# opendilab/DI-engine

Measured on NVIDIA H100. Metric: learner transitions/sec (GAE+ppo_error fwd+bwd, T=128 x B=4096 per GPU), higher is better.
Workload: dtype f32

## Files before the change

### di-engine_b200/csrc/policy.cu

```cuda
#include <math.h>

#include "../../include/b200rl.h"
#include "policy_stats.cuh"

namespace b200rl {

constexpr int GS_NT = 1024;
constexpr int GS_MAX_T = 24576;

template <int VN>
__global__ void __launch_bounds__(GS_NT) gae_seq_kernel(const float* __restrict__ value, float* __restrict__ next_value,
                                                       const float* __restrict__ reward, const float* __restrict__ done,
                                                       const float* __restrict__ traj, float* __restrict__ adv, int T,
                                                       float gamma, float gl, int mask_inplace, RetArgs ra) {
    pdl_prologue();
    extern __shared__ float s_seq[];
    float* s_d = s_seq;
    float* s_f = s_seq + T;
    __shared__ int s_nseg;
    __shared__ int s_cnt[GS_NT / 32];
    const int tid = threadIdx.x;
    const float vs = ra.vscale;
    float mu = 0.f, sigma = 1.f;
    if constexpr (VN == VN_POPART) {
        mu = *ra.mu;
        sigma = *ra.sigma;
    }
    for (int t = tid; t < T; t += GS_NT) {
        const float v = vn_decode<VN>(value[t], vs);
        float nv = vn_decode<VN>(next_value[t], vs);
        float r = reward[t];
        if constexpr (VN == VN_POPART) r = __fdiv_rn(fsub(r, mu), sigma);
        const float d = done ? done[t] : 0.f;
        const float tf = traj ? traj[t] : d;
        if (done) {
            nv = fmul(nv, fsub(1.f, d));
            if (VN == VN_PPO && mask_inplace && d != 0.f) next_value[t] = nv;
        }
        s_d[t] = fsub(fadd(r, fmul(gamma, nv)), v);
        s_f[t] = fmul(gl, fsub(1.f, tf));
    }
    __syncthreads();
    const int strip = (T + GS_NT - 1) / GS_NT;
    const int t0 = tid * strip, t1 = min(T, t0 + strip);
    int mine = 0;
    for (int t = t0; t < t1; ++t) mine += (s_f[t] == 0.f || t == T - 1) ? 1 : 0;
    int incl = mine;
    const int lane = tid & 31, wid = tid >> 5;
#pragma unroll
    for (int o = 1; o < 32; o <<= 1) {
        const int n = __shfl_up_sync(0xffffffffu, incl, o);
        if (lane >= o) incl += n;
    }
    if (lane == 31) s_cnt[wid] = incl;
    __syncthreads();
    if (wid == 0) {
        int w = s_cnt[lane];
#pragma unroll
        for (int o = 1; o < 32; o <<= 1) {
            const int n = __shfl_up_sync(0xffffffffu, w, o);
            if (lane >= o) w += n;
        }
        s_cnt[lane] = w;
        if (lane == 31) s_nseg = w;
    }
    __syncthreads();
    const int base = incl - mine + (wid ? s_cnt[wid - 1] : 0);
    __shared__ int s_end[GS_NT];
    const int nseg = s_nseg;
    const bool fits = nseg <= GS_NT;
    if (fits) {
        int k = base;
        for (int t = t0; t < t1; ++t)
            if (s_f[t] == 0.f || t == T - 1) s_end[k++] = t;
    }
    __syncthreads();
    if (fits) {
        if (tid < nseg) {
            const int hi = s_end[tid];
            const int lo = tid ? s_end[tid - 1] + 1 : 0;
            float carry = 0.f;
            int t = hi;
            for (; t - 15 >= lo; t -= 16) {
                float d[16], f[16];
#pragma unroll
                for (int k = 0; k < 16; ++k) {
                    d[k] = s_d[t - k];
                    f[k] = s_f[t - k];
                }
#pragma unroll
                for (int k = 0; k < 16; ++k) {
                    carry = fadd(d[k], fmul(f[k], carry));
                    d[k] = carry;
                }
#pragma unroll
                for (int k = 0; k < 16; ++k) s_d[t - k] = d[k];
            }
            for (; t >= lo; --t) {
                carry = fadd(s_d[t], fmul(s_f[t], carry));
                s_d[t] = carry;
            }
        }
    } else if (tid == 0) {
        float carry = 0.f;
        for (int t = T - 1; t >= 0; --t) {
            carry = fadd(s_d[t], fmul(s_f[t], carry));
            s_d[t] = carry;
        }
    }
    __syncthreads();
    if constexpr (VN != VN_PPO) {
        __shared__ int s_cut;
        if (tid == 0) s_cut = -1;
        __syncthreads();
        int cut = -1;
        for (int t = tid; t < T - 1; t += GS_NT)
            if (s_f[t] == 0.f && !isfinite(s_d[t + 1])) cut = t;
        if (cut >= 0) atomicMax(&s_cut, cut);
        __syncthreads();
        const int c = s_cut;
        for (int t = tid; t <= c; t += GS_NT) s_d[t] = __int_as_float(0x7fc00000);
        __syncthreads();
    }
    double acc[4] = {0.0, 0.0, 0.0, 0.0}, pv[2];
    ret_pivots<VN>(vs, vn_decode<VN>(ld_after_wait(value), vs), s_d[0], pv);
    for (int t = tid; t < T; t += GS_NT) {
        const float a = s_d[t];
        adv[t] = a;
        moments_add(acc[2], acc[3], a, pv[1]);
        if (ra.ret_unnorm || ra.value_out || ra.ret_out || ra.stats) {
            float ru, vo, ro;
            moments_add(acc[0], acc[1], ret_encode<VN>(vs, vn_decode<VN>(value[t], vs), a, ru, vo, ro), pv[0]);
            if (ra.ret_unnorm) ra.ret_unnorm[t] = ru;
            if (ra.value_out) ra.value_out[t] = vo;
            if (ra.ret_out) ra.ret_out[t] = ro;
        }
    }
    if (ra.stats || ra.adv_stats) {
        double tot[4];
        if (stats_grid_join<4, GS_NT>(acc, tot, nullptr, nullptr)) write_ret_stats<VN>(ra, tot, pv, (double)T);
    }
}

template <int VN, bool VEC>
__global__ void __launch_bounds__(256) returns_kernel(const float* __restrict__ value, const float* __restrict__ adv,
                                                      long long n, RetArgs ra, double* __restrict__ ws_part,
                                                      unsigned int* __restrict__ ws_join) {
    pdl_prologue();
    const float vs = ra.vscale;
    double acc[4] = {0.0, 0.0, 0.0, 0.0}, pv[2];
    const long long stride = (long long)gridDim.x * 256;
    long long i = (long long)blockIdx.x * 256 + threadIdx.x;
    if (VEC) {
        const long long n4 = n >> 2;
        const float4* v4 = reinterpret_cast<const float4*>(value);
        const float4* a4 = reinterpret_cast<const float4*>(adv);
        float4 v = make_float4(0.f, 0.f, 0.f, 0.f), a = v;
        if (i < n4) {
            v = v4[i];
            a = a4[i];
        }
        ret_pivots<VN>(vs, ret_value<VN>(ld_after_wait(value), vs), ld_after_wait(adv), pv);
        for (; i < n4; i += stride) {
            float4 ru, vo, ro;
            ret_one<VN>(vs, v.x, a.x, ru.x, vo.x, ro.x, acc, pv);
            ret_one<VN>(vs, v.y, a.y, ru.y, vo.y, ro.y, acc, pv);
            ret_one<VN>(vs, v.z, a.z, ru.z, vo.z, ro.z, acc, pv);
            ret_one<VN>(vs, v.w, a.w, ru.w, vo.w, ro.w, acc, pv);
            if (ra.ret_unnorm) reinterpret_cast<float4*>(ra.ret_unnorm)[i] = ru;
            if (ra.value_out) reinterpret_cast<float4*>(ra.value_out)[i] = vo;
            if (ra.ret_out) reinterpret_cast<float4*>(ra.ret_out)[i] = ro;
            if (i + stride < n4) {
                v = v4[i + stride];
                a = a4[i + stride];
            }
        }
    } else {
        float v = 0.f, a = 0.f;
        if (i < n) {
            v = value[i];
            a = adv[i];
        }
        ret_pivots<VN>(vs, ret_value<VN>(ld_after_wait(value), vs), ld_after_wait(adv), pv);
        for (; i < n; i += stride) {
            float ru, vo, ro;
            ret_one<VN>(vs, v, a, ru, vo, ro, acc, pv);
            if (ra.ret_unnorm) ra.ret_unnorm[i] = ru;
            if (ra.value_out) ra.value_out[i] = vo;
            if (ra.ret_out) ra.ret_out[i] = ro;
            if (i + stride < n) {
                v = value[i + stride];
                a = adv[i + stride];
            }
        }
    }
    if (!ra.stats && !ra.adv_stats) return;
    double tot[4];
    if (stats_grid_join<4, 256>(acc, tot, ws_part, ws_join)) write_ret_stats<VN>(ra, tot, pv, (double)n);
}

__global__ void __launch_bounds__(256) adv_stats_kernel(const float* __restrict__ x, long long n, float* __restrict__ out,
                                                        double* __restrict__ ws_part, unsigned int* __restrict__ ws_join) {
    pdl_prologue();
    const double p = stats_pivot(ld_after_wait(x));
    double acc[2] = {0.0, 0.0};
    for (long long i = (long long)blockIdx.x * 256 + threadIdx.x; i < n; i += (long long)gridDim.x * 256)
        moments_add(acc[0], acc[1], x[i], p);
    double tot[2];
    if (stats_grid_join<2, 256>(acc, tot, ws_part, ws_join)) write_adv_stats(out, tot[0], tot[1], p, (double)n);
}

__global__ void __launch_bounds__(256) normalize_kernel(const float* __restrict__ x, const float* __restrict__ stats,
                                                        long long n, float* __restrict__ out) {
    pdl_prologue();
    const float m = ld_after_wait(stats), d = ld_after_wait(stats + 1);
    for (long long i = (long long)blockIdx.x * 256 + threadIdx.x; i < n; i += (long long)gridDim.x * 256)
        out[i] = __fdiv_rn(fsub(x[i], m), d);
}

__global__ void __launch_bounds__(256) impala_mask_kernel(const float* __restrict__ values, const float* __restrict__ rewards,
                                                          const float* __restrict__ done, long long T, long long B,
                                                          float* __restrict__ values_out, float* __restrict__ rewards_out,
                                                          float* __restrict__ weights_out) {
    pdl_prologue();
    const long long n = (T + 1) * B;
    for (long long i = (long long)blockIdx.x * 256 + threadIdx.x; i < n; i += (long long)gridDim.x * 256) {
        const long long t = i / B;
        const float m = t >= 1 ? fsub(1.f, done[i - B]) : 1.f;
        values_out[i] = t >= 1 ? fmul(values[i], m) : values[i];
        if (t < T) {
            if (weights_out) weights_out[i] = m;
            if (rewards_out) rewards_out[i] = fmul(rewards[i], m);
        }
    }
}

enum ValueMap : int { VM_SYMLOG = 0, VM_INV_SYMLOG = 1, VM_H_INV = 2, VM_POPART_REWARD = 3 };

template <int M>
__device__ __forceinline__ float value_map(float x, float mu, float sigma) {
    if constexpr (M == VM_SYMLOG) return vn_symlog(x);
    else if constexpr (M == VM_INV_SYMLOG) return vn_inv_symlog(x);
    else if constexpr (M == VM_H_INV) return vn_h_inv(x);
    else return __fdiv_rn(fsub(x, mu), sigma);
}

template <int M>
__global__ void __launch_bounds__(256) value_map_kernel(const float* __restrict__ x0, float* __restrict__ y0,
                                                        const float* __restrict__ x1, float* __restrict__ y1, long long n,
                                                        const float* __restrict__ mu, const float* __restrict__ sigma) {
    pdl_prologue();
    float m = 0.f, sg = 1.f;
    if constexpr (M == VM_POPART_REWARD) {
        m = *mu;
        sg = *sigma;
    }
    for (long long i = (long long)blockIdx.x * 256 + threadIdx.x; i < n; i += (long long)gridDim.x * 256) {
        y0[i] = value_map<M>(x0[i], m, sg);
        if (x1) y1[i] = value_map<M>(x1[i], m, sg);
    }
}

template <int M>
__global__ void __launch_bounds__(256) value_map_bwd_kernel(const float* __restrict__ x, const float* __restrict__ g,
                                                            float* __restrict__ dx, long long n) {
    pdl_prologue();
    for (long long i = (long long)blockIdx.x * 256 + threadIdx.x; i < n; i += (long long)gridDim.x * 256) {
        const float xi = x[i], s = vn_sign(xi), gs = fmul(g[i], s);
        const float d = M == VM_SYMLOG ? __fdiv_rn(gs, fadd(fabsf(xi), 1.f)) : fmul(gs, expf(fabsf(xi)));
        dx[i] = fadd(0.f, fmul(d, s));
    }
}

}

using namespace b200rl;

namespace b200rl {
int gae_scan(const float* value, float* next_value, const float* reward, const float* done, const float* traj_flag, float* adv,
             long long T, long long C, long long A, double gamma_d, double lambda_d, int mask_next_value_inplace,
             float vscale, void* stream);
}

static double* ws_stats_part(float* ws) { return reinterpret_cast<double*>(ws + WS_CTRL_WORDS); }
static unsigned int* ws_joins(float* ws) { return reinterpret_cast<unsigned int*>(ws + WS_FX_OFF_WORDS + 48); }
static_assert(WS_CTRL_WORDS % 2 == 0 && WS_CTRL_WORDS + NUM_SMS * 8 * 4 * 2 <= WS_PARTIAL_LIMIT_WORDS,
              "the statistics rows fit the workspace's partial region");

extern "C" int b200rl_adv_stats(const float* x, long long n, float* stats2, float* workspace, size_t workspace_bytes,
                                void* stream) {
    if (!x || !stats2 || !workspace || n < 1 || workspace_bytes < WS_MIN_BYTES) return B200RL_ERR_ARG;
    long long grid = div_up(n, 256 * 8);
    if (grid > NUM_SMS * 4) grid = NUM_SMS * 4;
    if (grid < 1) grid = 1;
    return launch_k(adv_stats_kernel, (int)grid, 256, 0, (cudaStream_t)stream, x, n, stats2, ws_stats_part(workspace),
                    ws_joins(workspace));
}

extern "C" int b200rl_normalize(const float* x, const float* stats2, long long n, float* out, void* stream) {
    if (!x || !stats2 || !out || n < 0) return B200RL_ERR_ARG;
    if (n == 0) return B200RL_OK;
    long long grid = div_up(n, 256 * 4);
    if (grid > NUM_SMS * 8) grid = NUM_SMS * 8;
    return launch_k(normalize_kernel, (int)grid, 256, 0, (cudaStream_t)stream, x, stats2, n, out);
}

extern "C" int b200rl_gae_returns(const float* value, float* next_value, const float* reward, const float* done,
                                  const float* traj_flag, long long T, long long C, long long A, double gamma,
                                  double lambda_, int mask_next_value_inplace, double value_scale, float* adv,
                                  float* unnormalized_return, float* value_out, float* return_out, float* stats3,
                                  float* adv_stats2, float* workspace, size_t workspace_bytes, void* stream) {
    if (T < 1 || C < 1 || A < 1 || !value || !next_value || !reward || !adv || !workspace ||
        workspace_bytes < WS_MIN_BYTES || value_scale < 0.0)
        return B200RL_ERR_ARG;
    RetArgs ra{};
    ra.vscale = (float)value_scale;
    ra.ret_unnorm = unnormalized_return; ra.value_out = value_out; ra.ret_out = return_out; ra.stats = stats3;
    ra.adv_stats = adv_stats2;
    cudaStream_t st = (cudaStream_t)stream;
    if (C == 1 && T <= GS_MAX_T) {
        const size_t smem = (size_t)2 * T * sizeof(float);
        if (int rc = smem_opt_in<gae_seq_kernel<VN_PPO>>(smem)) return rc;
        return launch_k(gae_seq_kernel<VN_PPO>, 1, GS_NT, smem, st, value, next_value, reward, done, traj_flag, adv, (int)T,
                        (float)gamma, (float)(gamma * lambda_), mask_next_value_inplace, ra);
    }
    const bool want_epi = unnormalized_return || value_out || return_out || stats3 || adv_stats2;
    int rc = gae_scan(value, next_value, reward, done, traj_flag, adv, T, C, A, gamma, lambda_, mask_next_value_inplace,
                      (float)value_scale, stream);
    if (rc != 0 || !want_epi) return rc;
    const long long n = T * C;
    const bool vec = (n % 4 == 0) && aligned16(value) && aligned16(adv) && (!unnormalized_return || aligned16(unnormalized_return)) &&
                     (!value_out || aligned16(value_out)) && (!return_out || aligned16(return_out));
    long long grid = div_up(n, 256 * (vec ? 8 : 4));
    if (grid > NUM_SMS * 8) grid = NUM_SMS * 8;
    if (vec)
        return launch_k(returns_kernel<VN_PPO, true>, (int)grid, 256, 0, st, value, (const float*)adv, n, ra,
                        ws_stats_part(workspace), ws_joins(workspace));
    return launch_k(returns_kernel<VN_PPO, false>, (int)grid, 256, 0, st, value, (const float*)adv, n, ra,
                    ws_stats_part(workspace), ws_joins(workspace));
}

static long long map_grid(long long n) {
    long long grid = div_up(n, 256 * 4);
    if (grid > NUM_SMS * 8) grid = NUM_SMS * 8;
    return grid < 1 ? 1 : grid;
}

template <int VN>
static int launch_gae_seq(const float* value, const float* next_value, const float* reward, const float* done,
                          const float* traj_flag, float* adv, long long T, double gamma, double lambda_, const RetArgs& ra,
                          cudaStream_t st) {
    const size_t smem = (size_t)2 * T * sizeof(float);
    if (int rc = smem_opt_in<gae_seq_kernel<VN>>(smem)) return rc;
    return launch_k(gae_seq_kernel<VN>, 1, GS_NT, smem, st, value, const_cast<float*>(next_value), reward, done, traj_flag,
                    adv, (int)T, (float)gamma, (float)(gamma * lambda_), 0, ra);
}

template <int VN>
static int launch_returns(const float* value, const float* adv, long long n, const RetArgs& ra, float* workspace,
                          cudaStream_t st) {
    const bool vec = (n % 4 == 0) && aligned16(value) && aligned16(adv) && (!ra.value_out || aligned16(ra.value_out)) &&
                     (!ra.ret_out || aligned16(ra.ret_out));
    long long grid = div_up(n, 256 * (vec ? 8 : 4));
    if (grid > NUM_SMS * 8) grid = NUM_SMS * 8;
    if (vec)
        return launch_k(returns_kernel<VN, true>, (int)grid, 256, 0, st, value, adv, n, ra, ws_stats_part(workspace),
                        ws_joins(workspace));
    return launch_k(returns_kernel<VN, false>, (int)grid, 256, 0, st, value, adv, n, ra, ws_stats_part(workspace),
                    ws_joins(workspace));
}

template <int VN>
static int launch_gae_returns_tc(const float* value, const float* next_value, const float* reward, const float* done,
                                 const float* traj_flag, float* adv, long long T, long long C, double gamma, double lambda_,
                                 const RetArgs& ra, float* scratch, float* workspace, cudaStream_t st) {
    const long long n = T * C;
    const float* v = value;
    const float* nv = next_value;
    const float* r = reward;
    int rc = 0;
    if constexpr (VN == VN_RESCALE || VN == VN_SYMLOG) {
        constexpr int M = VN == VN_RESCALE ? VM_H_INV : VM_INV_SYMLOG;
        rc = launch_k(value_map_kernel<M>, (int)map_grid(n), 256, 0, st, value, scratch, next_value, scratch + n, n,
                      (const float*)nullptr, (const float*)nullptr);
        v = scratch;
        nv = scratch + n;
    } else if constexpr (VN == VN_POPART) {
        rc = launch_k(value_map_kernel<VM_POPART_REWARD>, (int)map_grid(n), 256, 0, st, reward, scratch,
                      (const float*)nullptr, (float*)nullptr, n, ra.mu, ra.sigma);
        r = scratch;
    }
    if (rc) return rc;
    rc = gae_scan(v, const_cast<float*>(nv), r, done, traj_flag, adv, T, C, 1, gamma, lambda_, 0,
                  VN == VN_BASELINE ? ra.vscale : 0.f, st);
    if (rc || !(ra.value_out || ra.ret_out || ra.stats || ra.adv_stats)) return rc;
    return launch_returns<VN>(v, adv, n, ra, workspace, st);
}

template <int VN>
static int gae_returns_norm(const float* value, const float* next_value, const float* reward, const float* done,
                            const float* traj_flag, float* adv, long long T, long long C, double gamma, double lambda_,
                            const RetArgs& ra, float* scratch, float* workspace, cudaStream_t st) {
    if (C == 1 && T <= GS_MAX_T)
        return launch_gae_seq<VN>(value, next_value, reward, done, traj_flag, adv, T, gamma, lambda_, ra, st);
    return launch_gae_returns_tc<VN>(value, next_value, reward, done, traj_flag, adv, T, C, gamma, lambda_, ra, scratch,
                                     workspace, st);
}

extern "C" int b200rl_gae_returns_norm(const float* value, const float* next_value, const float* reward, const float* done,
                                       const float* traj_flag, long long T, long long C, double gamma, double lambda_,
                                       int value_norm, double std, const float* popart_mu, const float* popart_sigma,
                                       float* adv, float* value_out, float* return_out, float* stats3, float* adv_stats2,
                                       float* scratch, float* workspace, size_t workspace_bytes, void* stream) {
    if (T < 1 || C < 1 || !value || !next_value || !reward || !adv || !workspace || workspace_bytes < WS_MIN_BYTES)
        return B200RL_ERR_ARG;
    if (value_norm < VN_BASELINE || value_norm > VN_POPART) return B200RL_ERR_ARG;
    if (value_norm == VN_BASELINE && !(std > 0.0)) return B200RL_ERR_ARG;
    if (value_norm == VN_POPART && (!popart_mu || !popart_sigma)) return B200RL_ERR_ARG;
    const bool one_launch = C == 1 && T <= GS_MAX_T;
    if (!one_launch && value_norm != VN_BASELINE && !scratch) return B200RL_ERR_ARG;
    RetArgs ra{};
    ra.vscale = value_norm == VN_BASELINE ? (float)std : 0.f;
    ra.value_out = value_out; ra.ret_out = return_out; ra.stats = stats3; ra.adv_stats = adv_stats2;
    ra.mu = popart_mu; ra.sigma = popart_sigma;
    cudaStream_t st = (cudaStream_t)stream;
    switch (value_norm) {
        case VN_BASELINE:
            return gae_returns_norm<VN_BASELINE>(value, next_value, reward, done, traj_flag, adv, T, C, gamma, lambda_, ra,
                                                 scratch, workspace, st);
        case VN_RESCALE:
            return gae_returns_norm<VN_RESCALE>(value, next_value, reward, done, traj_flag, adv, T, C, gamma, lambda_, ra,
                                                scratch, workspace, st);
        case VN_SYMLOG:
            return gae_returns_norm<VN_SYMLOG>(value, next_value, reward, done, traj_flag, adv, T, C, gamma, lambda_, ra,
                                               scratch, workspace, st);
        default:
            return gae_returns_norm<VN_POPART>(value, next_value, reward, done, traj_flag, adv, T, C, gamma, lambda_, ra,
                                               scratch, workspace, st);
    }
}

extern "C" int b200rl_value_map_fwd(int mode, const float* x, long long n, float* y, void* stream) {
    if (n < 0 || (mode != VM_SYMLOG && mode != VM_INV_SYMLOG)) return B200RL_ERR_ARG;
    if (n == 0) return B200RL_OK;
    if (!x || !y) return B200RL_ERR_ARG;
    cudaStream_t st = (cudaStream_t)stream;
    const int grid = (int)map_grid(n);
    if (mode == VM_SYMLOG)
        return launch_k(value_map_kernel<VM_SYMLOG>, grid, 256, 0, st, x, y, (const float*)nullptr, (float*)nullptr, n,
                        (const float*)nullptr, (const float*)nullptr);
    return launch_k(value_map_kernel<VM_INV_SYMLOG>, grid, 256, 0, st, x, y, (const float*)nullptr, (float*)nullptr, n,
                    (const float*)nullptr, (const float*)nullptr);
}

extern "C" int b200rl_value_map_bwd(int mode, const float* x, const float* g, long long n, float* dx, void* stream) {
    if (n < 0 || (mode != VM_SYMLOG && mode != VM_INV_SYMLOG)) return B200RL_ERR_ARG;
    if (n == 0) return B200RL_OK;
    if (!x || !g || !dx) return B200RL_ERR_ARG;
    cudaStream_t st = (cudaStream_t)stream;
    const int grid = (int)map_grid(n);
    if (mode == VM_SYMLOG) return launch_k(value_map_bwd_kernel<VM_SYMLOG>, grid, 256, 0, st, x, g, dx, n);
    return launch_k(value_map_bwd_kernel<VM_INV_SYMLOG>, grid, 256, 0, st, x, g, dx, n);
}

extern "C" int b200rl_impala_mask(const float* values, const float* rewards, const float* done, long long T, long long B,
                                  float* values_out, float* rewards_out, float* weights_out, void* stream) {
    if (!values || !done || !values_out || T < 1 || B < 1 || (rewards_out && !rewards)) return B200RL_ERR_ARG;
    long long grid = div_up((T + 1) * B, 256 * 4);
    if (grid > NUM_SMS * 8) grid = NUM_SMS * 8;
    return launch_k(impala_mask_kernel, (int)grid, 256, 0, (cudaStream_t)stream, values, rewards, done, T, B, values_out,
                    rewards_out, weights_out);
}
```

### di-engine_b200/csrc/policy_stats.cuh

```cuda
#pragma once
#include <math.h>

#include "common.cuh"

namespace b200rl {

template <class T>
__device__ __forceinline__ T warp_sum_t(T v) {
#pragma unroll
    for (int o = 16; o > 0; o >>= 1) v += __shfl_xor_sync(0xffffffffu, v, o);
    return v;
}

template <int K, int NT>
__device__ __forceinline__ void block_sum_d(double (&v)[K], double (&tot)[K]) {
    __shared__ double s_bs[K][NT / 32];
    const int lane = threadIdx.x & 31, wid = threadIdx.x >> 5;
#pragma unroll
    for (int k = 0; k < K; ++k) {
        const double r = warp_sum_t(v[k]);
        if (lane == 0) s_bs[k][wid] = r;
    }
    __syncthreads();
    if (threadIdx.x == 0) {
#pragma unroll
        for (int k = 0; k < K; ++k) {
            double r = 0.0;
            for (int w = 0; w < NT / 32; ++w) r += s_bs[k][w];
            tot[k] = r;
        }
    }
    __syncthreads();
}

struct RetArgs {
    float vscale;
    float* ret_unnorm;
    float* value_out;
    float* ret_out;
    float* stats;
    float* adv_stats;
    const float* mu;
    const float* sigma;
};

enum ValueNorm : int { VN_BASELINE = 0, VN_RESCALE = 1, VN_SYMLOG = 2, VN_POPART = 3, VN_PPO = 4 };

__device__ __forceinline__ float vn_sign(float x) { return (float)((0.f < x) - (x < 0.f)); }

__device__ __forceinline__ float vn_h(float x) {
    return fadd(fmul(vn_sign(x), fsub(__fsqrt_rn(fadd(fabsf(x), 1.f)), 1.f)), fmul(0.01f, x));
}
__device__ __forceinline__ float vn_h_inv(float x) {
    const float u = __fdiv_rn(fsub(__fsqrt_rn(fadd(1.f, fmul(0.04f, fadd(fadd(fabsf(x), 1.f), 0.01f)))), 1.f), 0.02f);
    return fmul(vn_sign(x), fsub(fmul(u, u), 1.f));
}
__device__ __forceinline__ float vn_symlog(float x) { return fmul(vn_sign(x), logf(fadd(fabsf(x), 1.f))); }
__device__ __forceinline__ float vn_inv_symlog(float x) { return fmul(vn_sign(x), fsub(expf(fabsf(x)), 1.f)); }

template <int VN>
__device__ __forceinline__ float vn_decode(float v, float vs) {
    if constexpr (VN == VN_PPO || VN == VN_BASELINE) return vs != 0.f ? fmul(v, vs) : v;
    else if constexpr (VN == VN_RESCALE) return vn_h_inv(v);
    else if constexpr (VN == VN_SYMLOG) return vn_inv_symlog(v);
    else return v;
}

template <int VN>
__device__ __forceinline__ float vn_encode(float v, float vs) {
    if constexpr (VN == VN_PPO || VN == VN_BASELINE) return vs != 0.f ? __fdiv_rn(v, vs) : v;
    else if constexpr (VN == VN_RESCALE) return vn_h(v);
    else if constexpr (VN == VN_SYMLOG) return vn_symlog(v);
    else return v;
}

template <int VN>
__device__ __forceinline__ float ret_encode(float vs, float v, float a, float& ru, float& vo, float& ro) {
    const float r = fadd(v, a);
    ru = r;
    vo = vn_encode<VN>(v, vs);
    ro = vn_encode<VN>(r, vs);
    return VN == VN_PPO ? r : ro;
}

__device__ __forceinline__ double stats_pivot(float x0) { return isfinite(x0) ? (double)x0 : 0.0; }

__device__ __forceinline__ float ld_after_wait(const float* p) { return __ldcg(p); }

__device__ __forceinline__ void moments_add(double& s1, double& s2, float x, double p) {
    const double d = (double)x - p;
    s1 += d;
    s2 = fma(d, d, s2);
}

template <int VN>
__device__ __forceinline__ float ret_value(float v, float vs) {
    if constexpr (VN == VN_PPO || VN == VN_BASELINE) return vn_decode<VN>(v, vs);
    else return v;
}

template <int VN>
__device__ __forceinline__ void ret_one(float vs, float v, float a, float& ru, float& vo, float& ro, double (&acc)[4],
                                        const double (&pv)[2]) {
    moments_add(acc[0], acc[1], ret_encode<VN>(vs, ret_value<VN>(v, vs), a, ru, vo, ro), pv[0]);
    moments_add(acc[2], acc[3], a, pv[1]);
}

template <int VN>
__device__ __forceinline__ void ret_pivots(float vs, float v0, float a0, double (&pv)[2]) {
    float ru, vo, ro;
    pv[0] = stats_pivot(ret_encode<VN>(vs, v0, a0, ru, vo, ro));
    pv[1] = stats_pivot(a0);
}

template <int K, int NT>
__device__ __forceinline__ bool stats_grid_join(double (&acc)[K], double (&tot)[K], double* part, unsigned int* ticket) {
    __shared__ bool s_last;
    block_sum_d<K, NT>(acc, tot);
    if (gridDim.x == 1) return threadIdx.x == 0;
    if (threadIdx.x == 0) {
#pragma unroll
        for (int k = 0; k < K; ++k) part[(size_t)blockIdx.x * K + k] = tot[k];
        __threadfence();
        s_last = atomicAdd(ticket, 1u) == gridDim.x - 1;
    }
    __syncthreads();
    if (!s_last) return false;
    __threadfence();
    double v[K];
#pragma unroll
    for (int k = 0; k < K; ++k) v[k] = 0.0;
    for (unsigned int b = threadIdx.x; b < gridDim.x; b += NT)
#pragma unroll
        for (int k = 0; k < K; ++k) v[k] += __ldcg(part + (size_t)b * K + k);
    block_sum_d<K, NT>(v, tot);
    if (threadIdx.x == 0) *ticket = 0u;
    return threadIdx.x == 0;
}

__device__ __forceinline__ void write_adv_stats(float* out, double s1, double s2, double p, double nn) {
    const double d = s1 / nn;
    const double var = (s2 - s1 * d) / (nn - 1.0);
    const double sd = var != var ? var : sqrt(fmax(var, 0.0));
    out[0] = (float)(p + d);
    out[1] = fadd((float)sd, 1e-8f);
}

template <int VN>
__device__ __forceinline__ double pop_var(double v) {
    return (VN != VN_PPO && v != v) ? v : fmax(v, 0.0);
}

template <int VN>
__device__ __forceinline__ void write_ret_stats(const RetArgs& ra, const double (&tot)[4], const double (&pv)[2],
                                                double nn) {
    if (ra.stats) {
        const double d = tot[0] / nn;
        ra.stats[0] = (float)(pv[0] + d);
        ra.stats[1] = (float)pop_var<VN>(tot[1] / nn - d * d);
        ra.stats[2] = (float)nn;
    }
    if (ra.adv_stats) write_adv_stats(ra.adv_stats, tot[2], tot[3], pv[1], nn);
}

}
```

Baseline: 20.07 billion.

## Fuse GAE scan and returns epilogue into warp-specialized pipelined kernel

Adds a single persistent kernel that fuses the GAE backward scan with the returns/value/stats epilogue. A producer warp streams time chunks of column tiles into shared memory with cp.async and mbarriers, a scan warp computes deltas and carries the recurrence, and epilogue warps write adv, returns and accumulate moments. The goal is to remove the separate scan and epilogue passes and the global round trip of adv between them. It brings in a pivot-corrected grid stats join, since each CTA now uses its own pivot, and a serial single-warp scan per tile that could limit throughput.

```diff
diff --git a/di-engine_b200/csrc/policy.cu b/di-engine_b200/csrc/policy.cu
--- a/di-engine_b200/csrc/policy.cu
+++ b/di-engine_b200/csrc/policy.cu
@@ -199,6 +199,165 @@
     if (stats_grid_join<4, 256>(acc, tot, ws_part, ws_join)) write_ret_stats<VN>(ra, tot, pv, (double)n);
 }
 
+constexpr int GR_CH = 256;
+constexpr int GR_STAGES = 8;
+constexpr int GR_EW = 2;
+constexpr int GR_THREADS = (GR_EW + 2) * 32;
+constexpr int GR_CTAS_PER_SM = 2;
+static_assert(GR_EW * 32 * 4 == GR_CH, "one float4 of the chunk per epilogue thread");
+
+template <int TC>
+__global__ void __launch_bounds__(GR_THREADS) gae_returns_ws_kernel(
+    const float* __restrict__ value, float* __restrict__ next_value, const float* __restrict__ reward,
+    const float* __restrict__ done, const float* __restrict__ traj, float* __restrict__ adv, long long T, long long C,
+    float gamma, float gl, int mask_inplace, RetArgs ra, double* __restrict__ ws_part, unsigned int* __restrict__ ws_join) {
+    constexpr int R = GR_CH / TC, PR = TC / 4;
+    pdl_prologue();
+    __shared__ __align__(16) float s_raw[GR_STAGES][5][GR_CH];
+    __shared__ __align__(8) uint64_t s_full[GR_STAGES], s_ready[GR_STAGES], s_empty[GR_STAGES];
+    const int tid = threadIdx.x, wid = tid >> 5, lane = tid & 31;
+    if (tid == 0) {
+        for (int s = 0; s < GR_STAGES; ++s) {
+            mbar_init(&s_full[s], 32);
+            mbar_init(&s_ready[s], 1);
+            mbar_init(&s_empty[s], GR_EW);
+        }
+        mbar_fence_init();
+    }
+    __syncthreads();
+    const long long n_tiles = (C + TC - 1) / TC, n_chunks = (T + R - 1) / R;
+    const bool has_done = done != nullptr, has_traj = traj != nullptr;
+    const float vs = ra.vscale;
+    long long tile = blockIdx.x, q = 0;
+    int s = 0, ph = 0;
+    auto next = [&]() {
+        if (++s == GR_STAGES) { s = 0; ph ^= 1; }
+        if (++q == n_chunks) { q = 0; tile += gridDim.x; }
+    };
+    double acc[4] = {0.0, 0.0, 0.0, 0.0}, pv[2] = {0.0, 0.0};
+
+    if (wid == GR_EW) {
+        for (int j = 0; tile < n_tiles; ++j, next()) {
+            if (j >= GR_STAGES) mbar_wait(&s_empty[s], (uint32_t)(ph ^ 1));
+            const long long c0 = tile * TC, t0 = T - (q + 1) * R;
+            const long long W = C - c0 < TC ? C - c0 : TC;
+#pragma unroll
+            for (int k = 0; k < 2; ++k) {
+                const int p = lane + 32 * k, row = p / PR, o = (p % PR) * 4;
+                if (t0 + row >= 0 && o < W) {
+                    const long long off = (t0 + row) * C + c0 + o;
+                    cpa16(&s_raw[s][0][p * 4], value + off);
+                    cpa16(&s_raw[s][1][p * 4], next_value + off);
+                    cpa16(&s_raw[s][2][p * 4], reward + off);
+                    if (has_done) cpa16(&s_raw[s][3][p * 4], done + off);
+                    if (has_traj) cpa16(&s_raw[s][4][p * 4], traj + off);
+                }
+            }
+            cpa_mbar_arrive(&s_full[s]);
+        }
+    } else if (wid == GR_EW + 1) {
+        float carry = 0.f;
+        for (; tile < n_tiles; next()) {
+            mbar_wait(&s_full[s], (uint32_t)ph);
+            if (q == 0) carry = 0.f;
+            const long long c0 = tile * TC, t0 = T - (q + 1) * R;
+            const long long W = C - c0 < TC ? C - c0 : TC;
+            float* sv = s_raw[s][0];
+            float* sn = s_raw[s][1];
+            float* sr = s_raw[s][2];
+#pragma unroll
+            for (int k = 0; k < 2; ++k) {
+                const int p = lane + 32 * k, row = p / PR, o = (p % PR) * 4;
+                const long long t = t0 + row;
+                if (t >= 0 && o < W) {
+                    const float4 v4 = *reinterpret_cast<const float4*>(sv + p * 4);
+                    const float4 n4 = *reinterpret_cast<const float4*>(sn + p * 4);
+                    const float4 r4 = *reinterpret_cast<const float4*>(sr + p * 4);
+                    const float4 d4 = has_done ? *reinterpret_cast<const float4*>(&s_raw[s][3][p * 4])
+                                               : make_float4(0.f, 0.f, 0.f, 0.f);
+                    const float4 t4 = has_traj ? *reinterpret_cast<const float4*>(&s_raw[s][4][p * 4]) : d4;
+                    float vv[4] = {v4.x, v4.y, v4.z, v4.w}, nn[4] = {n4.x, n4.y, n4.z, n4.w};
+                    const float rw[4] = {r4.x, r4.y, r4.z, r4.w}, dd[4] = {d4.x, d4.y, d4.z, d4.w};
+                    const float tt[4] = {t4.x, t4.y, t4.z, t4.w};
+                    float de[4], fa[4];
+                    bool changed = false;
+#pragma unroll
+                    for (int e = 0; e < 4; ++e) {
+                        if (vs != 0.f) {
+                            vv[e] = fmul(vv[e], vs);
+                            nn[e] = fmul(nn[e], vs);
+                        }
+                        if (has_done) {
+                            changed |= (dd[e] != 0.f);
+                            nn[e] = fmul(nn[e], fsub(1.f, dd[e]));
+                        }
+                        de[e] = fsub(fadd(rw[e], fmul(gamma, nn[e])), vv[e]);
+                        fa[e] = fmul(gl, fsub(1.f, tt[e]));
+                    }
+                    *reinterpret_cast<float4*>(sr + p * 4) = make_float4(de[0], de[1], de[2], de[3]);
+                    *reinterpret_cast<float4*>(sn + p * 4) = make_float4(fa[0], fa[1], fa[2], fa[3]);
+                    if (changed && mask_inplace)
+                        *reinterpret_cast<float4*>(next_value + t * C + c0 + o) = make_float4(nn[0], nn[1], nn[2], nn[3]);
+                }
+            }
+            __syncwarp();
+            if (lane < W) {
+                if (t0 >= 0) {
+                    float d[R], f[R];
+#pragma unroll
+                    for (int k = 0; k < R; ++k) {
+                        d[k] = sr[(R - 1 - k) * TC + lane];
+                        f[k] = sn[(R - 1 - k) * TC + lane];
+                    }
+#pragma unroll
+                    for (int k = 0; k < R; ++k) {
+                        carry = fadd(d[k], fmul(f[k], carry));
+                        sr[(R - 1 - k) * TC + lane] = carry;
+                    }
+                } else {
+                    for (int jj = R - 1; jj >= 0 && t0 + jj >= 0; --jj) {
+                        carry = fadd(sr[jj * TC + lane], fmul(sn[jj * TC + lane], carry));
+                        sr[jj * TC + lane] = carry;
+                    }
+                }
+            }
+            __syncwarp();
+            if (lane == 0) mbar_arrive(&s_ready[s]);
+        }
+    } else {
+        const int p = tid, row = p / PR, o = (p % PR) * 4;
+        for (int j = 0; tile < n_tiles; ++j, next()) {
+            mbar_wait(&s_ready[s], (uint32_t)ph);
+            const float* sv = s_raw[s][0];
+            const float* sa = s_raw[s][2];
+            if (j == 0) ret_pivots<VN_PPO>(vs, vn_decode<VN_PPO>(sv[(R - 1) * TC], vs), sa[(R - 1) * TC], pv);
+            const long long c0 = tile * TC, t = T - (q + 1) * R + row;
+            if (t >= 0 && c0 + o < C) {
+                const float4 v = *reinterpret_cast<const float4*>(sv + p * 4);
+                const float4 a = *reinterpret_cast<const float4*>(sa + p * 4);
+                float4 ru, vo, ro;
+                ret_one<VN_PPO>(vs, v.x, a.x, ru.x, vo.x, ro.x, acc, pv);
+                ret_one<VN_PPO>(vs, v.y, a.y, ru.y, vo.y, ro.y, acc, pv);
+                ret_one<VN_PPO>(vs, v.z, a.z, ru.z, vo.z, ro.z, acc, pv);
+                ret_one<VN_PPO>(vs, v.w, a.w, ru.w, vo.w, ro.w, acc, pv);
+                const long long off = t * C + c0 + o;
+                *reinterpret_cast<float4*>(adv + off) = a;
+                if (ra.ret_unnorm) *reinterpret_cast<float4*>(ra.ret_unnorm + off) = ru;
+                if (ra.value_out) *reinterpret_cast<float4*>(ra.value_out + off) = vo;
+                if (ra.ret_out) *reinterpret_cast<float4*>(ra.ret_out + off) = ro;
+            }
+            __syncwarp();
+            if (lane == 0) mbar_arrive(&s_empty[s]);
+        }
+    }
+    if (!ra.stats && !ra.adv_stats) return;
+    double n = 0.0;
+    for (long long tl = blockIdx.x; tl < n_tiles; tl += gridDim.x) n += (double)T * (double)(C - tl * TC < TC ? C - tl * TC : TC);
+    double tot[4];
+    if (stats_grid_join_pivots<2, GR_THREADS>(acc, pv, n, tot, ws_part, ws_join))
+        write_ret_stats<VN_PPO>(ra, tot, pv, (double)T * (double)C);
+}
+
 __global__ void __launch_bounds__(256) adv_stats_kernel(const float* __restrict__ x, long long n, float* __restrict__ out,
                                                         double* __restrict__ ws_part, unsigned int* __restrict__ ws_join) {
     pdl_prologue();
@@ -284,8 +443,35 @@
 
 static double* ws_stats_part(float* ws) { return reinterpret_cast<double*>(ws + WS_CTRL_WORDS); }
 static unsigned int* ws_joins(float* ws) { return reinterpret_cast<unsigned int*>(ws + WS_FX_OFF_WORDS + 48); }
-static_assert(WS_CTRL_WORDS % 2 == 0 && WS_CTRL_WORDS + NUM_SMS * 8 * 4 * 2 <= WS_PARTIAL_LIMIT_WORDS,
+static_assert(WS_CTRL_WORDS % 2 == 0 && WS_CTRL_WORDS + NUM_SMS * 8 * 7 * 2 <= WS_PARTIAL_LIMIT_WORDS,
               "the statistics rows fit the workspace's partial region");
+
+template <int TC>
+static int launch_gae_returns_ws_tc(const float* value, float* next_value, const float* reward, const float* done,
+                                    const float* traj_flag, float* adv, long long T, long long C, float gamma, float gl,
+                                    int mask_inplace, const RetArgs& ra, float* workspace, int sm_count, cudaStream_t st) {
+    const long long n_tiles = (C + TC - 1) / TC;
+    const long long grid = n_tiles < (long long)sm_count * GR_CTAS_PER_SM ? n_tiles : (long long)sm_count * GR_CTAS_PER_SM;
+    return launch_k(gae_returns_ws_kernel<TC>, (int)grid, GR_THREADS, 0, st, value, next_value, reward, done, traj_flag, adv,
+                    T, C, gamma, gl, mask_inplace, ra, ws_stats_part(workspace), ws_joins(workspace));
+}
+
+static int launch_gae_returns_ws(const float* value, float* next_value, const float* reward, const float* done,
+                                 const float* traj_flag, float* adv, long long T, long long C, float gamma, float gl,
+                                 int mask_inplace, const RetArgs& ra, float* workspace, cudaStream_t st) {
+    int sm_count = 0, per_sm = 0;
+    if (int rc = resident_ctas<gae_returns_ws_kernel<32>>(GR_THREADS, 0, sm_count, per_sm)) return rc;
+    if (sm_count > NUM_SMS * 4) sm_count = NUM_SMS * 4;
+    const long long enough = sm_count - sm_count / 16;
+    if ((C + 31) / 32 >= enough)
+        return launch_gae_returns_ws_tc<32>(value, next_value, reward, done, traj_flag, adv, T, C, gamma, gl, mask_inplace,
+                                            ra, workspace, sm_count, st);
+    if ((C + 15) / 16 >= enough)
+        return launch_gae_returns_ws_tc<16>(value, next_value, reward, done, traj_flag, adv, T, C, gamma, gl, mask_inplace,
+                                            ra, workspace, sm_count, st);
+    return launch_gae_returns_ws_tc<8>(value, next_value, reward, done, traj_flag, adv, T, C, gamma, gl, mask_inplace, ra,
+                                       workspace, sm_count, st);
+}
 
 extern "C" int b200rl_adv_stats(const float* x, long long n, float* stats2, float* workspace, size_t workspace_bytes,
                                 void* stream) {
@@ -325,6 +511,12 @@
                         (float)gamma, (float)(gamma * lambda_), mask_next_value_inplace, ra);
     }
     const bool want_epi = unnormalized_return || value_out || return_out || stats3 || adv_stats2;
+    if (want_epi && A == 1 && C % 4 == 0 && aligned16(value) && aligned16(next_value) && aligned16(reward) && aligned16(adv) &&
+        (!done || aligned16(done)) && (!traj_flag || aligned16(traj_flag)) &&
+        (!unnormalized_return || aligned16(unnormalized_return)) && (!value_out || aligned16(value_out)) &&
+        (!return_out || aligned16(return_out)))
+        return launch_gae_returns_ws(value, next_value, reward, done, traj_flag, adv, T, C, (float)gamma,
+                                     (float)(gamma * lambda_), mask_next_value_inplace, ra, workspace, st);
     int rc = gae_scan(value, next_value, reward, done, traj_flag, adv, T, C, A, gamma, lambda_, mask_next_value_inplace,
                       (float)value_scale, stream);
     if (rc != 0 || !want_epi) return rc;
diff --git a/di-engine_b200/csrc/policy_stats.cuh b/di-engine_b200/csrc/policy_stats.cuh
--- a/di-engine_b200/csrc/policy_stats.cuh
+++ b/di-engine_b200/csrc/policy_stats.cuh
@@ -138,6 +138,51 @@
     return threadIdx.x == 0;
 }
 
+template <int NS, int NT>
+__device__ __forceinline__ bool stats_grid_join_pivots(double (&acc)[2 * NS], double (&pv)[NS], double n,
+                                                       double (&tot)[2 * NS], double* part, unsigned int* ticket) {
+    constexpr int K = 2 * NS, ROW = 1 + NS + K;
+    __shared__ bool s_last;
+    block_sum_d<K, NT>(acc, tot);
+    if (gridDim.x == 1) return threadIdx.x == 0;
+    if (threadIdx.x == 0) {
+        double* row = part + (size_t)blockIdx.x * ROW;
+        row[0] = n;
+#pragma unroll
+        for (int i = 0; i < NS; ++i) row[1 + i] = pv[i];
+#pragma unroll
+        for (int k = 0; k < K; ++k) row[1 + NS + k] = tot[k];
+        __threadfence();
+        s_last = atomicAdd(ticket, 1u) == gridDim.x - 1;
+    }
+    __syncthreads();
+    if (!s_last) return false;
+    __threadfence();
+    double P[NS], v[K];
+#pragma unroll
+    for (int i = 0; i < NS; ++i) P[i] = __ldcg(part + 1 + i);
+#pragma unroll
+    for (int k = 0; k < K; ++k) v[k] = 0.0;
+    for (unsigned int b = threadIdx.x; b < gridDim.x; b += NT) {
+        const double* row = part + (size_t)b * ROW;
+        const double nb = __ldcg(row);
+#pragma unroll
+        for (int i = 0; i < NS; ++i) {
+            const double d = __ldcg(row + 1 + i) - P[i];
+            const double s1 = __ldcg(row + 1 + NS + 2 * i), s2 = __ldcg(row + 2 + NS + 2 * i);
+            v[2 * i] += s1 + nb * d;
+            v[2 * i + 1] += s2 + d * (2.0 * s1 + nb * d);
+        }
+    }
+    block_sum_d<K, NT>(v, tot);
+    if (threadIdx.x == 0) {
+        *ticket = 0u;
+#pragma unroll
+        for (int i = 0; i < NS; ++i) pv[i] = P[i];
+    }
+    return threadIdx.x == 0;
+}
+
 __device__ __forceinline__ void write_adv_stats(float* out, double s1, double s2, double p, double nn) {
     const double d = s1 / nn;
     const double var = (s2 - s1 * d) / (nn - 1.0);
```

Result: no change. 20.10 billion (median of 6 runs) (+0.1%).
